# lauraset/Super-resolution-building-height-estimation

Hardware: AMD Instinct MI355X
Metric: tiles/sec (64x64x8ch->256x256 height) (higher is better)
Workload: dtype f16 operands / f32 accumulate (MFMA), f32 residual stream; 1 GPU; RRDBNet x4 (23 RRDB, 64 feat) forward_feature, batch 32 tiles/GPU, 64x64x3 -> 64x256x256 (BASELINE.json configs[1]); global_batch=32, parallelism=tile-sharded x1 (no data-path collective)

## Files before the change

super-resolution-building-height-estimation_amd/csrc/srbh_aux.hip:

```cpp
#include "srbh_internal.h"

namespace srbh {

static thread_local char g_err[512] = "";

unsigned long long g_path_counters[PATH_N] = {};
void set_error(const char* fmt, ...) {
    va_list ap;
    va_start(ap, fmt);
    vsnprintf(g_err, sizeof(g_err), fmt, ap);
    va_end(ap);
}

int hip_fail(hipError_t e, const char* what) {
    set_error("HIP error %d (%s) in %s", (int)e, hipGetErrorString(e), what);
    return (int)e;
}

__global__ void zero_words_kernel(unsigned* __restrict__ p, size_t n) {
    size_t i = (size_t)blockIdx.x * blockDim.x + threadIdx.x;
    const size_t stride = (size_t)gridDim.x * blockDim.x;
    for (; i < n; i += stride) p[i] = 0u;
}

// ... 129 lines not shown
        } else {
            const _Float16 h = (_Float16)v;
            hv[j] = __builtin_bit_cast(unsigned short, h);
        }
    }
    char* o = dst + (long)b * img_b + (long)(chunk0 + (o8 >> 2)) * plane_b + (long)(y + 1) * row_b + (x + 1) * PIX_B + (o8 & 3) * 16;
    uint4 pk = {(unsigned)hv[0] | ((unsigned)hv[1] << 16), (unsigned)hv[2] | ((unsigned)hv[3] << 16),
                (unsigned)hv[4] | ((unsigned)hv[5] << 16), (unsigned)hv[6] | ((unsigned)hv[7] << 16)};
    *(uint4*)o = pk;
}

template <int BF>
__global__ __launch_bounds__(256) void act16_channel_sum_kernel(const char* __restrict__ src, int B, int H, int W, int nchunk, int row_b,
                                                                 int plane_b, long img_b, float* __restrict__ out ) {
    __shared__ float red[32];
    if (threadIdx.x < 32) red[threadIdx.x] = 0.f;
    __syncthreads();
    const int oct = threadIdx.x & 3, pl = threadIdx.x >> 2;
    const int chunk = blockIdx.y;
    const long npix = (long)B * H * W;
    float acc[8] = {0.f, 0.f, 0.f, 0.f, 0.f, 0.f, 0.f, 0.f};
    for (long px = (long)blockIdx.x * 64 + pl; px < npix; px += (long)gridDim.x * 64) {
        const int x = (int)(px % W);
        const long r = px / W;
        const int y = (int)(r % H), b = (int)(r / H);
        const uint4 v = *(const uint4*)(src + (long)b * img_b + (long)chunk * plane_b + (long)(y + 1) * row_b + (x + 1) * PIX_B + oct * 16);
        const unsigned w4[4] = {v.x, v.y, v.z, v.w};
#pragma unroll
        for (int k = 0; k < 4; ++k) {
            if constexpr (BF) {
                acc[2 * k] += __builtin_bit_cast(float, w4[k] << 16);
                acc[2 * k + 1] += __builtin_bit_cast(float, w4[k] & 0xffff0000u);
            } else {
                acc[2 * k] += (float)__builtin_bit_cast(_Float16, (unsigned short)(w4[k] & 0xffffu));
                acc[2 * k + 1] += (float)__builtin_bit_cast(_Float16, (unsigned short)(w4[k] >> 16));
            }
        }
    }
#pragma unroll
    for (int k = 0; k < 8; ++k) {
        float a = acc[k];
#pragma unroll
        for (int m = 4; m < 64; m <<= 1) a += __shfl_xor(a, m);
        if ((threadIdx.x & 63) < 4) atomicAdd(&red[oct * 8 + k], a);
    }
    __syncthreads();
    if (threadIdx.x < 32) atomicAdd(out + chunk * 32 + threadIdx.x, red[threadIdx.x]);
}

template <int CIN, int BF16 = 0>
__global__ __launch_bounds__(256) void conv_first_kernel(const float* __restrict__ x, const float* __restrict__ w,
                                                         const float* __restrict__ bias, int B, int cin_rt, int H, int W,
                                                         float* ra, float* rb, float* rc, char* out16, int row_b,
                                                         int plane_b, long img_b) {
    extern __shared__ float s_w[];
    const int cin = CIN > 0 ? CIN : cin_rt;
    for (int u = threadIdx.x; u < cin * 9 * 64; u += 256) {
        const int oc = u & 63, k = u >> 6;
        s_w[u] = w[(long)oc * cin * 9 + k];
    }
    __syncthreads();
    const int wq = (W + 3) >> 2;
    const long idx = (long)blockIdx.x * 256 + threadIdx.x;
    const long total = (long)B * H * wq * 16;
    if (idx >= total) return;
    const int og = idx & 15;
    long r = idx >> 4;
    const int xg = r % wq; r /= wq;
    const int yy = r % H;
    const int b = r / H;
    const int x0 = xg * 4;
    float acc[4][4];
#pragma unroll
    for (int p = 0; p < 4; ++p)
#pragma unroll
        for (int q = 0; q < 4; ++q) acc[p][q] = bias ? bias[og * 4 + q] : 0.f;
    for (int ic = 0; ic < cin; ++ic) {
        const float* xp = x + ((long)b * cin + ic) * H * W;
#pragma unroll
        for (int ky = 0; ky < 3; ++ky) {
            const int sy = yy + ky - 1;
            float in[6];
#pragma unroll
            for (int j = 0; j < 6; ++j) {
                const int sx = x0 + j - 1;
                in[j] = (sy >= 0 && sy < H && sx >= 0 && sx < W) ? xp[(long)sy * W + sx] : 0.f;
            }
#pragma unroll
            for (int kx = 0; kx < 3; ++kx) {
                const float4 wv = *(const float4*)(s_w + (ic * 9 + ky * 3 + kx) * 64 + og * 4);
#pragma unroll
                for (int p = 0; p < 4; ++p) {
                    const float v = in[p + kx];
                    acc[p][0] = fmaf(v, wv.x, acc[p][0]);
                    acc[p][1] = fmaf(v, wv.y, acc[p][1]);
                    acc[p][2] = fmaf(v, wv.z, acc[p][2]);
                    acc[p][3] = fmaf(v, wv.w, acc[p][3]);
                }
            }
        }
    }
#pragma unroll
    for (int p = 0; p < 4; ++p) {
        const int xx = x0 + p;
        if (xx >= W) break;
        const long pix = ((long)b * H + yy) * W + xx;
        const float4 v4 = make_float4(acc[p][0], acc[p][1], acc[p][2], acc[p][3]);
        if (ra) *(float4*)(ra + pix * 64 + og * 4) = v4;
        if (rb) *(float4*)(rb + pix * 64 + og * 4) = v4;
// ... 201 lines not shown
            float4 row = {0.f, 0.f, 0.f, 0.f};
#pragma unroll
            for (int q = 0; q < 4; ++q) {
                const int gx = min(max(2 * ix - 1 + q, 0), 2 * W - 1);
                const float4 v = p[((long)gy * 2 * W + gx) * C4];
                row.x += wt[q] * v.x; row.y += wt[q] * v.y; row.z += wt[q] * v.z; row.w += wt[q] * v.w;
            }
            s.x += wt[a] * row.x; s.y += wt[a] * row.y; s.z += wt[a] * row.z; s.w += wt[a] * row.w;
        }
        dx[i] = s;
    }
}

extern "C" int srbh_bilinear2x_nhwc_f32(const float* x, float* out, int B, int H, int W, int C, int backward, void* stream) {
    SRBH_REQUIRE(x && out && B > 0 && H > 0 && W > 0 && C > 0 && (C & 3) == 0, "srbh_bilinear2x_nhwc_f32: bad arguments (C %% 4 == 0)");
    const long n4 = (long)B * H * W * (C / 4) * (backward ? 1 : 4);
    const int blocks = (int)((n4 + 255) / 256 < 8192 ? (n4 + 255) / 256 : 8192);
    if (backward) hipLaunchKernelGGL(bilinear2x_bwd_kernel, dim3(blocks), dim3(256), 0, (hipStream_t)stream, (const float4*)x, (float4*)out, n4, H, W, C / 4);
    else hipLaunchKernelGGL(bilinear2x_fwd_kernel, dim3(blocks), dim3(256), 0, (hipStream_t)stream, (const float4*)x, (float4*)out, n4, H, W, C / 4);
    SRBH_HIP(hipGetLastError());
    return SRBH_OK;
}

extern "C" int srbh_lrelu_bwd_f32(float* g, const float* y, float slope, long n, void* stream) {
    SRBH_REQUIRE(g && y && n > 0 && (n & 3) == 0, "srbh_lrelu_bwd_f32: bad arguments");
    const long n4 = n / 4;
    const int blocks = (int)((n4 + 255) / 256 < 4096 ? (n4 + 255) / 256 : 4096);
    hipLaunchKernelGGL(lrelu_bwd_kernel, dim3(blocks), dim3(256), 0, (hipStream_t)stream, (float4*)g, (const float4*)y, slope, n4);
    SRBH_HIP(hipGetLastError());
    return SRBH_OK;
}

extern "C" int srbh_act16_channel_sum(const void* src, int B, int H, int W, int chunks_total, int chunk0, int nchunk, int bf16, float* out,
                                      void* stream) {
    SRBH_REQUIRE(src && out && B > 0 && H > 0 && W > 0 && nchunk > 0 && chunk0 >= 0 && chunk0 + nchunk <= chunks_total, "srbh_act16_channel_sum: bad arguments");
    const Act16Geo g = act16_geo(B, chunks_total, H, W);
    if (int rc = zero_async(out, (size_t)nchunk * 32 * sizeof(float), (hipStream_t)stream)) return rc;
    const long npix = (long)B * H * W;
    const int gx = (int)((npix + 255) / 256 < 1024 ? (npix + 255) / 256 : 1024);
    const char* base = (const char*)src + (long)chunk0 * g.plane_b;
    if (bf16) hipLaunchKernelGGL(act16_channel_sum_kernel<1>, dim3(gx, nchunk), dim3(256), 0, (hipStream_t)stream, base, B, H, W, nchunk, g.row_b, g.plane_b, g.img_b, out);
    else hipLaunchKernelGGL(act16_channel_sum_kernel<0>, dim3(gx, nchunk), dim3(256), 0, (hipStream_t)stream, base, B, H, W, nchunk, g.row_b, g.plane_b, g.img_b, out);
    SRBH_HIP(hipGetLastError());
    return SRBH_OK;
}

extern "C" int srbh_conv_first_f32(const float* x, const float* w, const float* bias, int B, int cin, int H, int W,
                                   float* ra, float* rb, float* rc, void* out16, int out16_chunks_total,
                                   void* stream) {
    return srbh::conv_first_f32(x, w, bias, B, cin, H, W, ra, rb, rc, out16, out16_chunks_total, 0, stream);
}

int srbh::conv_first_f32(const float* x, const float* w, const float* bias, int B, int cin, int H, int W, float* ra, float* rb, float* rc,
                         void* out16, int out16_chunks_total, int bf16, void* stream) {
    SRBH_REQUIRE(x && w && B > 0 && cin > 0 && H > 0 && W > 0, "srbh_conv_first_f32: bad arguments");
    SRBH_REQUIRE(!out16 || out16_chunks_total >= 2, "srbh_conv_first_f32: out16 needs >= 2 chunk planes");
    Act16Geo g = act16_geo(B, out16_chunks_total > 0 ? out16_chunks_total : 2, H, W);
    SRBH_REQUIRE(cin <= 56, "srbh_conv_first_f32: at most 56 input channels (got %d)", cin);
    long total = (long)B * H * ((W + 3) / 4) * 16;
    const size_t lds = (size_t)cin * 9 * 64 * sizeof(float);
    if (cin == 3 && bf16)
        hipLaunchKernelGGL((conv_first_kernel<3, 1>), dim3((total + 255) / 256), dim3(256), lds, (hipStream_t)stream, x, w, bias,
                           B, cin, H, W, ra, rb, rc, (char*)out16, g.row_b, g.plane_b, g.img_b);
    else if (cin == 3)
        hipLaunchKernelGGL(conv_first_kernel<3>, dim3((total + 255) / 256), dim3(256), lds, (hipStream_t)stream, x, w, bias,
                           B, cin, H, W, ra, rb, rc, (char*)out16, g.row_b, g.plane_b, g.img_b);
    else if (bf16) {
        if (lds > 65536)
            SRBH_ONCE_PER_DEVICE(SRBH_HIP(hipFuncSetAttribute((const void*)conv_first_kernel<0, 1>, hipFuncAttributeMaxDynamicSharedMemorySize, 56 * 9 * 64 * 4)));
        hipLaunchKernelGGL((conv_first_kernel<0, 1>), dim3((total + 255) / 256), dim3(256), lds, (hipStream_t)stream, x, w, bias,
                           B, cin, H, W, ra, rb, rc, (char*)out16, g.row_b, g.plane_b, g.img_b);
    } else {
        if (lds > 65536)
            SRBH_ONCE_PER_DEVICE(SRBH_HIP(hipFuncSetAttribute((const void*)conv_first_kernel<0>, hipFuncAttributeMaxDynamicSharedMemorySize, 56 * 9 * 64 * 4)));
        hipLaunchKernelGGL(conv_first_kernel<0>, dim3((total + 255) / 256), dim3(256), lds, (hipStream_t)stream, x, w, bias,
                           B, cin, H, W, ra, rb, rc, (char*)out16, g.row_b, g.plane_b, g.img_b);
    }
    SRBH_HIP(hipGetLastError());
    return SRBH_OK;
}
```

super-resolution-building-height-estimation_amd/csrc/srbh_internal.h:

```cpp
#pragma once
#include <hip/hip_runtime.h>
#include <stdarg.h>
#include <stdio.h>
#include <type_traits>
#include <vector>
#include "srbh.h"

namespace srbh {

constexpr int PIX_B = 64;
constexpr int CHUNK_C = 32;
constexpr int TILE_W = 64;
constexpr int TILE_H = 8;

void set_error(const char* fmt, ...);
enum PathCounter { PATH_HCONV16 = 0, PATH_HCONV_TEMPLATE, PATH_ENTRY_FUSED, PATH_ENTRY_SPLIT, PATH_WGRAD16, PATH_WGRAD_B16_GENERIC,
                   PATH_WGRAD_F32, PATH_WGRAD_ENTRY_FUSED, PATH_WGRAD_ENTRY_SPLIT, PATH_HCONV_UP, PATH_HBWD16, PATH_HBLOCK16, PATH_N };
extern unsigned long long g_path_counters[PATH_N];
inline void count_path(int i) { ++g_path_counters[i]; }
int hconv16_wgs_cap();
int hconv_up_wgs_cap();
int hconv_entry_wgs_cap();
int hblock16_wgs_cap();
int hwgrad16_wgs_cap();
// ... 23 lines not shown
        if (!((done_ >> (dev_ & 63)) & 1ull)) {           \
            stmt;                                         \
            done_ |= 1ull << (dev_ & 63);                 \
        }                                                 \
    } while (0)

template <class P>
inline void head_set_tiles(P& p, int B, int H, int W, int th) {
    p.B = B; p.H = H; p.W = W;
    p.tiles_x = (W + TILE_W - 1) / TILE_W;
    p.tiles_per_img = p.tiles_x * ((H + th - 1) / th);
    p.ntiles = p.tiles_per_img * B;
    p.tiles_per_xcd = (p.ntiles + 7) / 8;
}
template <class P>
inline int head_walk_grid(const P& p, int cap) { return (p.tiles_per_xcd < cap / 8 ? p.tiles_per_xcd : cap / 8) * 8; }
template <int N, class F>
inline int with_const(int v, F&& f) {
    if constexpr (N == 1) return f(std::integral_constant<int, 0>{});
    else return v == N - 1 ? f(std::integral_constant<int, N - 1>{}) : with_const<N - 1>(v, f);
}
template <auto Kernel, bool RAISE_LDS = false, class P>
inline int launch(dim3 grid, int lds_bytes, hipStream_t st, const P& p) {
    if constexpr (RAISE_LDS)
        SRBH_ONCE_PER_DEVICE(SRBH_HIP(hipFuncSetAttribute((const void*)Kernel, hipFuncAttributeMaxDynamicSharedMemorySize, lds_bytes)));
    hipLaunchKernelGGL(Kernel, grid, dim3(256), lds_bytes, st, p);
    SRBH_HIP(hipGetLastError());
    return SRBH_OK;
}

struct Act16Geo {
    int row_b;
    int plane_b;
    long img_b;
    size_t total_b;
};
inline Act16Geo act16_geo(int B, int chunks, int H, int W) {
    Act16Geo g;
    g.row_b = (W + 2) * PIX_B;
    g.plane_b = (H + 2) * g.row_b;
    g.img_b = (long)chunks * g.plane_b;
    size_t slack = (size_t)(TILE_H + 4) * (size_t)((W + 2 > TILE_W + 2) ? (W + 2) : (TILE_W + 2)) * PIX_B + 8192;
    g.total_b = (size_t)B * g.img_b + slack;
    g.total_b = (g.total_b + 255) & ~(size_t)255;
    return g;
}


size_t ptrunk_aux_bytes(int B, int tiles_per_img);
size_t ptrunk_err_offset(int B, int tiles_per_img);
int ptail_run(const srbh_conv3x3_args* a, hipStream_t stream, int* used);
int ptail_wgs_cap();
int ptrunk_takes(int num_block, int H, int W, int* takes, int* ncu_out);
int ptrunk_run(const srbh_rrdbnet_desc* d, void* dense0, void* dense1, float* xr, float* xrr, int B, int H, int W,
               void* aux, hipStream_t stream, int* used, int* final_cur, long train_stride = 0, const void* mask = nullptr, long mask_stride = 0,
               bool bf16 = false);
int conv3x3_trunk_b16(const srbh_conv3x3_args* a, int out_f16, void* stream);
int conv_first_f32(const float* x, const float* w, const float* bias, int B, int cin, int H, int W, float* ra, float* rb, float* rc,
                   void* out16, int out16_chunks_total, int bf16, void* stream);


#if defined(__HIP_DEVICE_COMPILE__) || defined(__HIPCC__)
__device__ __forceinline__ void fold_stat_slots(double* stats, const int C, const int clear, double* red, double& s, double& q) {
    constexpr int NS = 64;
    const int t = threadIdx.x, V = 2 * C, G = 256 / V, v = t % V, g = t / V;
    double part = 0.0;
    if (g < G) {
        for (int k = g; k < NS; k += G) part += stats[(long)k * V + v];
        if (clear)
            for (int k = g; k < NS; k += G) stats[(long)k * V + v] = 0.0;
        red[g * V + v] = part;
    }
    __syncthreads();
    s = 0.0;
    q = 0.0;
    if (t < C)
        for (int k = 0; k < G; ++k) {
            s += red[k * V + t];
            q += red[k * V + C + t];
        }
}

__device__ __forceinline__ unsigned bf16x2_rne(float lo, float hi) {
    typedef float f2_t __attribute__((ext_vector_type(2)));
    typedef __bf16 b2_t __attribute__((ext_vector_type(2)));
    const f2_t f = {lo, hi};
    return __builtin_bit_cast(unsigned, __builtin_convertvector(f, b2_t));
}
#endif
}
```

super-resolution-building-height-estimation_amd/csrc/srbh_ptail.hip:

```cpp
#include "srbh_ptail_kernel.h"

namespace {
using namespace srbh;
using namespace srbh_k;

struct TParams {
    In16 in;
    const char* w;
    const float* bias;
    int H, W;
    int tiles_x, tiles_per_img, ntiles, tiles_per_wg;
    int lrelu;
    Out16 out16;
    float* out32;
};

constexpr int LRELU_RT = 2, OUT_16 = 1, OUT_32 = 2, OUT_RT = 3;
template <int UPS, int FULL>
constexpr int LDS_B = TAIL_LDS_B<UPS> + (FULL && UPS ? 2 * TileGeo<UPS>::UNITS * 16 : 0);

template <int UPS, int LRELU, int OUT, int FULL>
__global__ __launch_bounds__(256, 1) void ptail_kernel(const TParams p) {
    static_assert(FULL ? (LRELU != LRELU_RT && OUT != OUT_RT) : (LRELU == LRELU_RT && OUT == OUT_RT), "one general form, the rest full-tile forms");
    using G = TileGeo<UPS>;
// ... 166 lines not shown
                        for (int g = 0; g < 4; ++g) {
                            const floatx4 v = value(mb, i, g);
                            half4 h4;
#pragma unroll
                            for (int q = 0; q < 4; ++q) h4[q] = (_Float16)v[q];
                            const uint2 u = __builtin_bit_cast(uint2, h4);
                            hp[g][0] = u.x;
                            hp[g][1] = u.y;
                        }
#pragma unroll
                        for (int m = 0; m < 2; ++m) *(uintx4*)(o + (long)i * o16.row_b + (long)mb * o16.plane_b + m * 32) = pair16(hp[2 * m], hp[2 * m + 1]);
                    }
            }
            continue;
        }
        const int X = X0 + wc * 32 + l31;
#pragma unroll
        for (int i = 0; i < 4; ++i) {
            const int Y = Y0 + wr * 4 + i;
            const bool valid = (Y < p.H) && (X < p.W);
            const long pix = ((long)img * p.H + Y) * p.W + X;
#pragma unroll
            for (int mb = 0; mb < CB; ++mb) {
                unsigned hp[4][2];
#pragma unroll
                for (int g = 0; g < 4; ++g) {
                    floatx4 v;
#pragma unroll
                    for (int q = 0; q < 4; ++q) v[q] = acc[mb][i][g * 4 + q];
                    v += bias4[mb][g];
                    if (p.lrelu) {
#pragma unroll
                        for (int q = 0; q < 4; ++q) v[q] = v[q] >= 0.f ? v[q] : v[q] * 0.2f;
                    }
                    if (p.out32 && valid) *(floatx4*)(p.out32 + pix * 64 + mb * 32 + g * 8 + hi * 4) = v;
                    half4 h4;
#pragma unroll
                    for (int q = 0; q < 4; ++q) h4[q] = (_Float16)v[q];
                    const uint2 u = __builtin_bit_cast(uint2, h4);
                    hp[g][0] = u.x;
                    hp[g][1] = u.y;
                }
                if (p.out16.base) {
#pragma unroll
                    for (int m = 0; m < 2; ++m) {
                        store16_pair(p.out16, valid, img, mb, Y, X, m, hi, hp[2 * m], hp[2 * m + 1]);
                    }
                }
            }
        }
    }
}

thread_local int g_ptail_wgs_cap = 0;

thread_local int g_ptail_form_counts[SRBH_PTAIL_FORMS] = {};

template <int UPS, int LRELU, int OUT, int FULL>
int launch(const TParams& p0, hipStream_t stream) {
    static_assert(LDS_B<UPS, FULL> <= 163840, "resident weights + the input chunks must fit the 160 KiB LDS");
    constexpr auto kernel = ptail_kernel<UPS, LRELU, OUT, FULL>;
    constexpr int lds_b = LDS_B<UPS, FULL>;
    SRBH_ONCE_PER_DEVICE(SRBH_HIP(hipFuncSetAttribute((const void*)kernel, hipFuncAttributeMaxDynamicSharedMemorySize, lds_b)));
    TParams p = p0;
    int grid = 0;
    if (const int rc = tail_grid(p.ntiles, &p.tiles_per_wg, &grid)) return rc;
    hipLaunchKernelGGL(kernel, dim3(grid), dim3(256), lds_b, stream, p);
    SRBH_HIP(hipGetLastError());
    ++g_ptail_form_counts[FULL ? 1 + 4 * UPS + 2 * LRELU + (OUT == OUT_32) : 0];
    return SRBH_OK;
}

}

extern "C" int srbh_ptail_wgs_cap(int cap) {
    const int prev = g_ptail_wgs_cap;
    g_ptail_wgs_cap = cap > 0 ? cap : 0;
    return prev;
}

extern "C" int srbh_ptail_form_counts(int* counts, int n, int reset) {
    for (int i = 0; counts && i < n && i < SRBH_PTAIL_FORMS; ++i) counts[i] = g_ptail_form_counts[i];
    if (reset) for (int i = 0; i < SRBH_PTAIL_FORMS; ++i) g_ptail_form_counts[i] = 0;
    return SRBH_PTAIL_FORMS;
}

namespace srbh {

int ptail_wgs_cap() { return g_ptail_wgs_cap; }

int ptail_run(const srbh_conv3x3_args* a, hipStream_t stream, int* used) {
    *used = 0;
    const char* e = getenv("SRBH_PTAIL");
    if (e && e[0] == '0') return SRBH_OK;
    if (a->in_chunks != 2 || a->cout != 64 || a->res1 || a->res2 || a->skip) return SRBH_OK;
    if (a->out32 && a->out32_c != 64) return SRBH_OK;
    const int tiles_x = (a->W + TILE_W - 1) / TILE_W, tiles_y = (a->H + TILE_H - 1) / TILE_H;
    if (a->out16_nhwc && (!a->out16 || a->out32)) return SRBH_OK;
    if ((long)tiles_x * tiles_y * a->B < 512 && !a->out16_nhwc) return SRBH_OK;
    TParams p{};
    p.in = tail_in16(a, a->in, a->in_chunks_total, a->in_chunk0);
    p.w = (const char*)a->w;
    p.bias = a->bias;
    p.H = a->H;
    p.W = a->W;
    p.tiles_x = tiles_x;
    p.tiles_per_img = tiles_x * tiles_y;
    p.ntiles = p.tiles_per_img * a->B;
    p.lrelu = a->lrelu;
    p.out16 = tail_out16(a, a->out16, a->out16_chunks_total, a->out16_chunk0);
    p.out32 = a->out32;
    const bool full = a->H % TILE_H == 0 && a->W % TILE_W == 0 && (p.out16.base != nullptr) != (p.out32 != nullptr);
    const int rc = with_const<2>(a->upsample2x != 0, [&](auto u) {
        constexpr int UPS = decltype(u)::value;
        if (!full) return launch<UPS, LRELU_RT, OUT_RT, 0>(p, stream);
        return with_const<2>(a->lrelu != 0, [&](auto l) {
            return with_const<2>(p.out32 != nullptr, [&](auto o) { return launch<UPS, decltype(l)::value, decltype(o)::value ? OUT_32 : OUT_16, 1>(p, stream); });
        });
    });
    if (rc == SRBH_OK) *used = 1;
    return rc;
}

}
```

super-resolution-building-height-estimation_amd/csrc/srbh_ptrunk.hip:

```cpp
#include <stdlib.h>
#include <string.h>
#include <mutex>
#include "srbh_conv3x3_kernel.h"


namespace {
using namespace srbh;
using namespace srbh_k;

struct PLayer {
    const char* w;
    const float* bias;
};

struct PParams {
    char* dense[2];
    long img_b;
    int plane_b, row_b;
    float* xr;
    float* xrr;
    const PLayer* layers;
    int nlayers;
    int H, W, tiles_per_img, nblocks;
    int* prog;
    int* err;
    int* xcc;
    int force_wt;
    unsigned long long* prof;
    long dense_stride;
    int keep_all;
    int out_pixel;
    const char* mask;
    long mask_stride;
};

constexpr unsigned SPIN_LIMIT = 4u << 20;
using G = TileGeo<0>;
constexpr int IN_EX = G::UNITS * 16;
constexpr int A_STAGE_B = IN_EX + 18 * 1024, B_STAGE_B = IN_EX + 36 * 1024;
constexpr int A_BASE = IN_EX;
constexpr int A_BIAS_OFF = A_BASE + 2 * A_STAGE_B, B_BIAS_OFF = 2 * B_STAGE_B;
constexpr int P_WORD_OFF = A_BIAS_OFF + 128;
constexpr int P_LDS_B = 163840;
static_assert(P_WORD_OFF + 4 <= P_LDS_B && B_BIAS_OFF + 256 <= P_WORD_OFF, "LDS map must fit 160 KiB");
__device__ __forceinline__ int stage_off(int cb, int idx) { return cb == 1 ? A_BASE + idx * A_STAGE_B : idx * B_STAGE_B; }

#include "srbh_ptrunk3_kernel.h"

}

namespace srbh {

unsigned long long* g_ptrunk_prof = nullptr;
static int g_trunk_timing = 0;
static hipEvent_t g_trunk_ev[2];
static int g_trunk_ev_recorded = 0;
static const char* g_trunk_kernel = "none";

constexpr int MAX_BLOCKS = 64;
static size_t table_bytes() { return ((size_t)MAX_BLOCKS * 15 * sizeof(PLayer) + 255) & ~(size_t)255; }
static size_t prog_bytes(int B, int tpi) { return ((size_t)B * 2 * tpi * sizeof(int) + 255) & ~(size_t)255; }

size_t ptrunk_aux_bytes(int B, int tiles_per_img) { return table_bytes() + 2 * prog_bytes(B, tiles_per_img) + 256; }
__global__ void ptrunk_reset_kernel(int* __restrict__ prog, int* __restrict__ xcc, int* __restrict__ err, int n) {
    const int i = blockIdx.x * blockDim.x + threadIdx.x;
    if (i < n) { prog[i] = 0; xcc[i] = 0; }
    if (i == 0) *err = 0;
}

size_t ptrunk_err_offset(int B, int tiles_per_img) { return table_bytes() + prog_bytes(B, tiles_per_img); }

struct TabEntry {
    int dev;
    std::vector<char> host;
    PLayer* dptr;
};
static std::mutex g_tab_mu;
static std::vector<TabEntry> g_tabs;

static int device_table(const std::vector<PLayer>& tab, PLayer** out) {
    int dev = 0;
    SRBH_HIP(hipGetDevice(&dev));
    const size_t nb = tab.size() * sizeof(PLayer);
    std::lock_guard<std::mutex> lock(g_tab_mu);
    for (size_t i = 0; i < g_tabs.size(); ++i)
        if (g_tabs[i].dev == dev && g_tabs[i].host.size() == nb && memcmp(g_tabs[i].host.data(), tab.data(), nb) == 0) {
            *out = g_tabs[i].dptr;
            return SRBH_OK;
        }
    if (g_tabs.size() >= 16) {
        SRBH_HIP(hipFree(g_tabs.front().dptr));
        g_tabs.erase(g_tabs.begin());
    }
    TabEntry e;
    e.dev = dev;
    e.host.assign((const char*)tab.data(), (const char*)tab.data() + nb);
    SRBH_HIP(hipMalloc(&e.dptr, nb));
    SRBH_HIP(hipMemcpy(e.dptr, tab.data(), nb, hipMemcpyHostToDevice));
    *out = e.dptr;
    g_tabs.push_back(std::move(e));
    return SRBH_OK;
}

int ptrunk_takes(int num_block, int H, int W, int* takes, int* ncu_out) {
    *takes = 0;
    if (W != TILE_W || (H % TILE_H) != 0 || num_block <= 0 || num_block > MAX_BLOCKS) return SRBH_OK;
    int dev = 0;
    SRBH_HIP(hipGetDevice(&dev));
    int ncu = 0;
    SRBH_HIP(hipDeviceGetAttribute(&ncu, hipDeviceAttributeMultiprocessorCount, dev));
    if (ncu_out) *ncu_out = ncu;
    if (H / TILE_H > ncu) return SRBH_OK;
    constexpr int LDS_B = P_LDS_B;
    SRBH_ONCE_PER_DEVICE({
        SRBH_HIP(hipFuncSetAttribute((const void*)ptrunk3_kernel<0>, hipFuncAttributeMaxDynamicSharedMemorySize, LDS_B));
        SRBH_HIP(hipFuncSetAttribute((const void*)ptrunk3_kernel<1>, hipFuncAttributeMaxDynamicSharedMemorySize, LDS_B));
        SRBH_HIP(hipFuncSetAttribute((const void*)ptrunk3_kernel<0, 1>, hipFuncAttributeMaxDynamicSharedMemorySize, LDS_B));
        SRBH_HIP(hipFuncSetAttribute((const void*)ptrunk3_kernel<0, 0, 1>, hipFuncAttributeMaxDynamicSharedMemorySize, LDS_B));
    });
    int per_cu = 0;
    SRBH_HIP(hipOccupancyMaxActiveBlocksPerMultiprocessor(&per_cu, ptrunk3_kernel<0>, 256, LDS_B));
    if (per_cu < 1) return SRBH_OK;
    *takes = 1;
    return SRBH_OK;
}

int ptrunk_run(const srbh_rrdbnet_desc* d, void* dense0, void* dense1, float* xr, float* xrr, int B, int H, int W,
               void* aux, hipStream_t stream, int* used, int* final_cur, long train_stride, const void* mask, long mask_stride, bool bf16) {
    *used = 0;
    if (mask && train_stride <= 0) return SRBH_OK;
    SRBH_REQUIRE(!bf16 || (train_stride == 0 && !mask), "ptrunk_run: the bf16 form is the inference forward only");
    int ncu = 0, takes = 0;
    if (int rc = ptrunk_takes(d->num_block, H, W, &takes, &ncu)) return rc;
    if (!takes) return SRBH_OK;
    const int tpi = H / TILE_H;
    constexpr int LDS_B = P_LDS_B;
    const int nl = d->num_block * 15;
    std::vector<PLayer> tab(nl);
    int cur = 0, li = 0;
    for (int blk = 0; blk < d->num_block; ++blk)
        for (int r = 0; r < 3; ++r) {
            const srbh_conv_w* cw = d->rdb + (blk * 3 + r) * 5;
            for (int k = 0; k < 5; ++k) tab[li++] = PLayer{(const char*)cw[k].w, cw[k].bias};
            cur ^= 1;
        }
    *final_cur = cur;
    char* a = (char*)aux;
    PLayer* d_tab = nullptr;
    if (int rc = device_table(tab, &d_tab)) return rc;
    int* d_prog = (int*)(a + table_bytes());
    int* d_err = (int*)(a + ptrunk_err_offset(B, tpi));
    int* d_xcc = (int*)(a + ptrunk_err_offset(B, tpi) + 256);
    hipLaunchKernelGGL(ptrunk_reset_kernel, dim3((B * tpi + 255) / 256), dim3(256), 0, stream, d_prog, d_xcc, d_err, B * tpi);
    SRBH_HIP(hipGetLastError());
    const Act16Geo g = act16_geo(B, 6, H, W);
    int imgs_per_launch = ncu / tpi;
    if (const char* ie = getenv("SRBH_PT_IMAGES")) {
        const int cap = atoi(ie);
        if (cap > 0 && cap < imgs_per_launch) {
            const int nl_ = (B + cap - 1) / cap;
            imgs_per_launch = (B + nl_ - 1) / nl_;
        }
    }
    for (int b0 = 0; b0 < B; b0 += imgs_per_launch) {
        const int nb = (B - b0) < imgs_per_launch ? (B - b0) : imgs_per_launch;
        PParams pp;
        pp.dense_stride = train_stride;
        pp.keep_all = pp.out_pixel = train_stride > 0;
        pp.mask = mask ? (const char*)mask + (long)b0 * g.img_b : nullptr;
        pp.mask_stride = mask_stride;
        pp.dense[0] = (char*)dense0 + (long)b0 * g.img_b;
        pp.dense[1] = (train_stride > 0 ? (char*)dense0 + train_stride : (char*)dense1) + (long)b0 * g.img_b;
        pp.img_b = g.img_b;
        pp.plane_b = g.plane_b;
        pp.row_b = g.row_b;
        pp.xr = xr + (long)b0 * H * W * 64;
        pp.xrr = xrr + (long)b0 * H * W * 64;
        pp.layers = d_tab;
        pp.nlayers = nl;
        pp.H = H;
        pp.W = W;
        pp.tiles_per_img = tpi;
        pp.nblocks = nb * tpi;
        pp.prog = d_prog + b0 * tpi;
        pp.err = d_err;
        pp.xcc = d_xcc + b0 * tpi;
        {
            const char* e = getenv("SRBH_PT_WT");
            pp.force_wt = (e && atoi(e) == 1) ? 1 : 0;
        }
        if (getenv("SRBH_PT_PROF") && !bf16 && !g_ptrunk_prof)
            SRBH_HIP(hipMalloc(&g_ptrunk_prof, (size_t)ncu * MAX_BLOCKS * 15 * 6 * 8));
        pp.prof = bf16 ? nullptr : g_ptrunk_prof;
        if (g_trunk_timing && b0 == 0) SRBH_HIP(hipEventRecord(g_trunk_ev[0], stream));
        g_trunk_kernel = "ptrunk3_kernel";
        if (mask)
            hipLaunchKernelGGL((ptrunk3_kernel<0, 1>), dim3(pp.nblocks), dim3(256), LDS_B, stream, pp);
        else if (bf16)
            hipLaunchKernelGGL((ptrunk3_kernel<0, 0, 1>), dim3(pp.nblocks), dim3(256), LDS_B, stream, pp);
        else if (pp.prof)
            hipLaunchKernelGGL((ptrunk3_kernel<1>), dim3(pp.nblocks), dim3(256), LDS_B, stream, pp);
        else
            hipLaunchKernelGGL((ptrunk3_kernel<0>), dim3(pp.nblocks), dim3(256), LDS_B, stream, pp);
        SRBH_HIP(hipGetLastError());
    }
    if (g_trunk_timing) { SRBH_HIP(hipEventRecord(g_trunk_ev[1], stream)); g_trunk_ev_recorded = 1; }
    if (getenv("SRBH_PT_PROF") && g_ptrunk_prof && !bf16) {
// ... 64 lines not shown
```

super-resolution-building-height-estimation_amd/csrc/srbh_rrdbnet.hip:

```cpp
#include <stdlib.h>
#include "srbh_internal.h"

using namespace srbh;

namespace {

struct WsLayout {
    size_t d0, d1, feat, xr, xrr, u2, u3, u4, aux, total;
    size_t u2lo, u3lo;
    size_t dense_b;
};

inline size_t align256(size_t v) { return (v + 255) & ~(size_t)255; }

__global__ __launch_bounds__(256) void poison_on_error_kernel(const int* __restrict__ err, float* __restrict__ out, size_t n) {
    if (__hip_atomic_load(err, __ATOMIC_RELAXED, __HIP_MEMORY_SCOPE_AGENT) == 0) return;
    const float nan = __builtin_nanf("");
    for (size_t i = (size_t)blockIdx.x * blockDim.x + threadIdx.x; i < n; i += (size_t)gridDim.x * blockDim.x) out[i] = nan;
}

__global__ __launch_bounds__(256) void trunk_out_pixel_order_kernel(const float* __restrict__ src, float* __restrict__ dst, long nquads) {
    typedef float f4 __attribute__((ext_vector_type(4)));
    for (long i = (long)blockIdx.x * blockDim.x + threadIdx.x; i < nquads; i += (long)gridDim.x * blockDim.x) {
        const long row = i >> 10;
// ... 91 lines not shown
    L.xr = off; off = align256(off + res_b);
    L.xrr = off; off = align256(off + res_b);
    L.u2 = off; off = align256(off + act16_geo(B, 2, 2 * H, 2 * W).total_b);
    L.u3 = off; off = align256(off + act16_geo(B, 2, 4 * H, 4 * W).total_b);
    L.u4 = off;
    if (want_forward == 1) off = align256(off + act16_geo(B, 2, 4 * H, 4 * W).total_b);
    L.aux = off;
    off = align256(off + ptrunk_aux_bytes(B, tiles_per_img(H)));
    L.u2lo = L.u3lo = off;
    if (f16x2) {
        L.u2lo = off; off = align256(off + act16_geo(B, 2, 2 * H, 2 * W).total_b);
        L.u3lo = off; off = align256(off + act16_geo(B, 2, 4 * H, 4 * W).total_b);
    }
    L.total = off;
    return L;
}

}

extern "C" size_t srbh_rrdbnet_workspace_bytes(int B, int H, int W, int want_forward) {
    if (B <= 0 || H <= 0 || W <= 0) return 0;
    return ws_layout(B, H, W, want_forward).total;
}

extern "C" size_t srbh_rrdbnet_workspace_bytes_f16x2(int B, int H, int W, int want_forward) {
    if (B <= 0 || H <= 0 || W <= 0) return 0;
    return ws_layout(B, H, W, want_forward, true).total;
}

extern "C" int srbh_rrdbnet_forward(const srbh_rrdbnet_desc* d, const float* x, float* out, int B, int H, int W,
                                    int want_forward, void* ws, size_t ws_bytes, void* stream) {
    SRBH_REQUIRE(d && x && out && ws, "srbh_rrdbnet_forward: null pointer");
    SRBH_REQUIRE(B > 0 && H > 0 && W > 0, "srbh_rrdbnet_forward: bad geometry B=%d H=%d W=%d", B, H, W);
    SRBH_REQUIRE(d->num_block >= 0 && d->rdb != nullptr, "srbh_rrdbnet_forward: bad descriptor");
    const bool split = d->tail_f16x2 != 0;
    SRBH_REQUIRE(!split || (d->conv_body_lo && d->conv_up1_lo && d->conv_up2_lo && d->conv_hr_lo),
                 "srbh_rrdbnet_forward: the f16x2 mode needs the lo' packs of conv_body, conv_up1, conv_up2 and conv_hr");
    SRBH_REQUIRE(!split || want_forward != 1, "srbh_rrdbnet_forward: the f16x2 mode computes forward_feature only (want_forward 0 or 2)");
    const WsLayout L = ws_layout(B, H, W, want_forward, split);
    if (ws_bytes < L.total) {
        set_error("srbh_rrdbnet_forward: workspace %zu bytes < required %zu", ws_bytes, L.total);
        return SRBH_ERR_WORKSPACE;
    }
    char* base = (char*)ws;
    void* D[2] = {base + L.d0, base + L.d1};
    float* feat = (float*)(base + L.feat);
    float* xr = (float*)(base + L.xr);
    float* xrr = (float*)(base + L.xrr);
    void* U2 = base + L.u2;
    void* U3 = base + L.u3;
    void* U4 = base + L.u4;

    const bool bf16 = d->rdb_b16 && d->num_block > 0 && !env_off("SRBH_TRUNK_BF16");
    int rc = conv_first_f32(x, d->conv_first_w, d->conv_first_b, B, d->num_in_ch, H, W, feat, xr, xrr, D[0], 6, bf16 ? 1 : 0, stream);
    if (rc) return rc;

    int cur = 0;
    int used_persistent = 0;
    if (!env_off("SRBH_PERSISTENT")) {
        srbh_rrdbnet_desc dt = *d;
        if (bf16) dt.rdb = d->rdb_b16;
        rc = ptrunk_run(&dt, D[0], D[1], xr, xrr, B, H, W, base + L.aux, (hipStream_t)stream, &used_persistent, &cur, 0, nullptr, 0, bf16);
        if (rc) return rc;
    }
    const int n_rdb = d->num_block * 3;
    for (int i = 0; !used_persistent && i < n_rdb; ++i) {
        const srbh_conv_w* cw = (bf16 ? d->rdb_b16 : d->rdb) + i * 5;
        if ((rc = run_rdb(D[cur], D[cur ^ 1], xr, i % 3 == 2 ? xrr : nullptr, cw, B, H, W, bf16, i + 1 == n_rdb, stream))) return rc;
        cur ^= 1;
    }

    void* U2lo = base + L.u2lo;
    void* U3lo = base + L.u3lo;
    if (split && (rc = srbh_act16_split_lo(xrr, used_persistent, D[cur], 6, 0, D[cur], 6, 2, B, H, W, stream))) return rc;
    srbh_conv3x3_args a = tail_conv(D[cur], 6, d->conv_body, B, H, W, 0, 0);
    a.skip = feat;
    out_planes(a, D[cur ^ 1], 6, 0);
    if ((rc = run_tail_conv(a, split, D[cur], 6, 2, d->conv_body_lo, D[cur ^ 1], 6, 2, stream))) return rc;
    a = tail_conv(D[cur ^ 1], 6, d->conv_up1, B, 2 * H, 2 * W, 1, 1);
    out_planes(a, U2, 2, 0);
    if ((rc = run_tail_conv(a, split, D[cur ^ 1], 6, 2, d->conv_up1_lo, U2lo, 2, 0, stream))) return rc;
    a = tail_conv(U2, 2, d->conv_up2, B, 4 * H, 4 * W, 1, 1);
    out_planes(a, U3, 2, 0);
    if ((rc = run_tail_conv(a, split, U2lo, 2, 0, d->conv_up2_lo, U3lo, 2, 0, stream))) return rc;
    a = tail_conv(U3, 2, d->conv_hr, B, 4 * H, 4 * W, 0, 0);
    const bool full = want_forward && want_forward != 2 && !split;
    int out_c = 64;
    if (want_forward == 2) {
        out_planes(a, out, 2, 0);
        a.out16_nhwc = 1;
        out_c = 32;
    } else if (!full) {
        a.out32 = out; a.out32_c = 64;
    } else {
        a.lrelu = 1;
        out_planes(a, U4, 2, 0);
    }
    if ((rc = run_tail_conv(a, split, U3lo, 2, 0, d->conv_hr_lo, nullptr, 0, 0, stream))) return rc;
    if (full) {
        SRBH_REQUIRE(d->conv_last.w && d->num_out_ch >= 1 && d->num_out_ch <= 32,
                     "srbh_rrdbnet_forward: conv_last needs 1..32 output channels (got %d)", d->num_out_ch);
        a = conv_on(U4, 2, 2, d->conv_last.w, d->conv_last.bias, 32, B, 4 * H, 4 * W);
        a.out32 = out; a.out32_c = out_c = d->num_out_ch;
        if ((rc = srbh_conv3x3_f16(&a, stream))) return rc;
    }
    if (!used_persistent) return SRBH_OK;
    return poison_on_error(ptrunk_err_word(base + L.aux, B, H), out, (size_t)B * 16 * H * W * out_c, 1024, (hipStream_t)stream);
}

extern "C" int srbh_rrdbnet_trunk_out(const void* ws, size_t ws_bytes, int num_block, int B, int H, int W, int want_forward, float* out,
                                      void* stream) {
    SRBH_REQUIRE(ws && out && B > 0 && H > 0 && W > 0 && num_block >= 0, "srbh_rrdbnet_trunk_out: bad arguments");
    const WsLayout L = ws_layout(B, H, W, want_forward);
    if (ws_bytes < L.total) {
        set_error("srbh_rrdbnet_trunk_out: workspace %zu bytes < required %zu", ws_bytes, L.total);
        return SRBH_ERR_WORKSPACE;
// ... 215 lines not shown
```

Baseline: 8555 tiles/s.

## Add pipelined conv_hr fp32 tail kernel and fold trunk reset into conv_first

Adds a dedicated fp32 full-tile kernel for the final conv_hr layer. It prefetches the next tile's input chunks partway through the MFMA loop and partway through the output store loop, so staging overlaps with compute and stores. The persistent-trunk progress, xcc and error-word reset is folded into the conv_first kernel, which removes a separate launch. conv_first also skips writing xr when the persistent trunk will run. Together these cut launch overhead and stalls on the tail layer, at the cost of a larger code path and a hard requirement that the persistent trunk accept the launch.

```diff
diff --git a/super-resolution-building-height-estimation_amd/csrc/srbh_aux.hip b/super-resolution-building-height-estimation_amd/csrc/srbh_aux.hip
--- a/super-resolution-building-height-estimation_amd/csrc/srbh_aux.hip
+++ b/super-resolution-building-height-estimation_amd/csrc/srbh_aux.hip
@@ -205,9 +205,14 @@
 __global__ __launch_bounds__(256) void conv_first_kernel(const float* __restrict__ x, const float* __restrict__ w,
                                                          const float* __restrict__ bias, int B, int cin_rt, int H, int W,
                                                          float* ra, float* rb, float* rc, char* out16, int row_b,
-                                                         int plane_b, long img_b) {
+                                                         int plane_b, long img_b, const PtrunkClear clr) {
     extern __shared__ float s_w[];
     const int cin = CIN > 0 ? CIN : cin_rt;
+    if (clr.n > 0) {
+        const long i = (long)blockIdx.x * 256 + threadIdx.x;
+        if (i < clr.n) { clr.prog[i] = 0; clr.xcc[i] = 0; }
+        if (i == 0) *clr.err = 0;
+    }
     for (int u = threadIdx.x; u < cin * 9 * 64; u += 256) {
         const int oc = u & 63, k = u >> 6;
         s_w[u] = w[(long)oc * cin * 9 + k];
@@ -515,30 +520,32 @@
 }
 
 int srbh::conv_first_f32(const float* x, const float* w, const float* bias, int B, int cin, int H, int W, float* ra, float* rb, float* rc,
-                         void* out16, int out16_chunks_total, int bf16, void* stream) {
+                         void* out16, int out16_chunks_total, int bf16, void* stream, const PtrunkClear* clear) {
     SRBH_REQUIRE(x && w && B > 0 && cin > 0 && H > 0 && W > 0, "srbh_conv_first_f32: bad arguments");
     SRBH_REQUIRE(!out16 || out16_chunks_total >= 2, "srbh_conv_first_f32: out16 needs >= 2 chunk planes");
     Act16Geo g = act16_geo(B, out16_chunks_total > 0 ? out16_chunks_total : 2, H, W);
     SRBH_REQUIRE(cin <= 56, "srbh_conv_first_f32: at most 56 input channels (got %d)", cin);
     long total = (long)B * H * ((W + 3) / 4) * 16;
     const size_t lds = (size_t)cin * 9 * 64 * sizeof(float);
+    const PtrunkClear clr = clear ? *clear : PtrunkClear{};
+    SRBH_REQUIRE(clr.n == 0 || (clr.prog && clr.xcc && clr.err && clr.n <= total), "srbh_conv_first_f32: bad clear words");
     if (cin == 3 && bf16)
         hipLaunchKernelGGL((conv_first_kernel<3, 1>), dim3((total + 255) / 256), dim3(256), lds, (hipStream_t)stream, x, w, bias,
-                           B, cin, H, W, ra, rb, rc, (char*)out16, g.row_b, g.plane_b, g.img_b);
+                           B, cin, H, W, ra, rb, rc, (char*)out16, g.row_b, g.plane_b, g.img_b, clr);
     else if (cin == 3)
         hipLaunchKernelGGL(conv_first_kernel<3>, dim3((total + 255) / 256), dim3(256), lds, (hipStream_t)stream, x, w, bias,
-                           B, cin, H, W, ra, rb, rc, (char*)out16, g.row_b, g.plane_b, g.img_b);
+                           B, cin, H, W, ra, rb, rc, (char*)out16, g.row_b, g.plane_b, g.img_b, clr);
     else if (bf16) {
         if (lds > 65536)
             SRBH_ONCE_PER_DEVICE(SRBH_HIP(hipFuncSetAttribute((const void*)conv_first_kernel<0, 1>, hipFuncAttributeMaxDynamicSharedMemorySize, 56 * 9 * 64 * 4)));
         hipLaunchKernelGGL((conv_first_kernel<0, 1>), dim3((total + 255) / 256), dim3(256), lds, (hipStream_t)stream, x, w, bias,
-                           B, cin, H, W, ra, rb, rc, (char*)out16, g.row_b, g.plane_b, g.img_b);
+                           B, cin, H, W, ra, rb, rc, (char*)out16, g.row_b, g.plane_b, g.img_b, clr);
     } else {
         if (lds > 65536)
             SRBH_ONCE_PER_DEVICE(SRBH_HIP(hipFuncSetAttribute((const void*)conv_first_kernel<0>, hipFuncAttributeMaxDynamicSharedMemorySize, 56 * 9 * 64 * 4)));
         hipLaunchKernelGGL(conv_first_kernel<0>, dim3((total + 255) / 256), dim3(256), lds, (hipStream_t)stream, x, w, bias,
-                           B, cin, H, W, ra, rb, rc, (char*)out16, g.row_b, g.plane_b, g.img_b);
-    }
-    SRBH_HIP(hipGetLastError());
-    return SRBH_OK;
-}
+                           B, cin, H, W, ra, rb, rc, (char*)out16, g.row_b, g.plane_b, g.img_b, clr);
+    }
+    SRBH_HIP(hipGetLastError());
+    return SRBH_OK;
+}
diff --git a/super-resolution-building-height-estimation_amd/csrc/srbh_internal.h b/super-resolution-building-height-estimation_amd/csrc/srbh_internal.h
--- a/super-resolution-building-height-estimation_amd/csrc/srbh_internal.h
+++ b/super-resolution-building-height-estimation_amd/csrc/srbh_internal.h
@@ -99,12 +99,19 @@
 int ptail_run(const srbh_conv3x3_args* a, hipStream_t stream, int* used);
 int ptail_wgs_cap();
 int ptrunk_takes(int num_block, int H, int W, int* takes, int* ncu_out);
+struct PtrunkClear {
+    int* prog = nullptr;
+    int* xcc = nullptr;
+    int* err = nullptr;
+    int n = 0;
+};
+PtrunkClear ptrunk_clear_words(void* aux, int B, int tiles_per_img);
 int ptrunk_run(const srbh_rrdbnet_desc* d, void* dense0, void* dense1, float* xr, float* xrr, int B, int H, int W,
                void* aux, hipStream_t stream, int* used, int* final_cur, long train_stride = 0, const void* mask = nullptr, long mask_stride = 0,
-               bool bf16 = false);
+               bool bf16 = false, bool cleared = false);
 int conv3x3_trunk_b16(const srbh_conv3x3_args* a, int out_f16, void* stream);
 int conv_first_f32(const float* x, const float* w, const float* bias, int B, int cin, int H, int W, float* ra, float* rb, float* rc,
-                   void* out16, int out16_chunks_total, int bf16, void* stream);
+                   void* out16, int out16_chunks_total, int bf16, void* stream, const PtrunkClear* clear = nullptr);
 
 
 #if defined(__HIP_DEVICE_COMPILE__) || defined(__HIPCC__)
diff --git a/super-resolution-building-height-estimation_amd/csrc/srbh_ptail.hip b/super-resolution-building-height-estimation_amd/csrc/srbh_ptail.hip
--- a/super-resolution-building-height-estimation_amd/csrc/srbh_ptail.hip
+++ b/super-resolution-building-height-estimation_amd/csrc/srbh_ptail.hip
@@ -242,14 +242,145 @@
     }
 }
 
+#ifndef PTAIL_LINES_SPLIT
+#define PTAIL_LINES_SPLIT 66
+#endif
+constexpr int LINES_STORES = 128, LINES_SPLIT = PTAIL_LINES_SPLIT;
+constexpr int LINES_YOUNGER = LINES_STORES - LINES_SPLIT < 63 ? LINES_STORES - LINES_SPLIT : 63;
+static_assert(LINES_SPLIT >= 0 && LINES_SPLIT < LINES_STORES && LINES_SPLIT % 2 == 0, "the two stores of a pixel record stay together");
+
+__global__ __launch_bounds__(256, 1) void ptail_hr32_lines(const TParams p) {
+    using G = TileGeo<0>;
+    constexpr int IN_EX = G::UNITS * 16;
+    constexpr int CB = 2;
+    extern __shared__ __attribute__((aligned(16))) char smem[];
+    const int tid = threadIdx.x;
+    const int lane = tid & 63;
+    const int wave = __builtin_amdgcn_readfirstlane(tid >> 6);
+    const int l31 = lane & 31, hi = lane >> 5;
+    const int wr = wave >> 1, wc = wave & 1;
+
+    int goff[G::NJ];
+#pragma unroll
+    for (int j = 0; j < G::NJ; ++j) {
+        const int u0 = j * 256 + tid;
+        const int u = u0 < G::UNITS ? u0 : 0;
+        const int trow = u / (G::COLS * 4);
+        const int rem = u - trow * (G::COLS * 4);
+        const int pc = rem >> 2, ps = rem & 3;
+        goff[j] = trow * p.in.row_b + pc * PIX_B + ((ps ^ ((pc >> 2) & 3)) << 4);
+    }
+    const unsigned long long tail_mask = __builtin_amdgcn_ballot_w64((G::NJ - 1) * 256 + tid < G::UNITS);
+    int aoff[3][2];
+#pragma unroll
+    for (int dx = 0; dx < 3; ++dx) {
+        const int pc = wc * 32 + l31 + dx;
+#pragma unroll
+        for (int ks = 0; ks < 2; ++ks) aoff[dx][ks] = wr * 4 * G::ROW_B + pc * PIX_B + (((ks * 2 + hi) ^ ((pc >> 2) & 3)) << 4);
+    }
+
+    auto stage_chunk = [&](int t, int c) {
+        int img, Y0, X0;
+        tile_origin(t, p.tiles_per_img, p.tiles_x, img, Y0, X0);
+        const char* src0 = p.in.base + (long)img * p.in.img_b + (long)Y0 * p.in.row_b + X0 * PIX_B;
+#pragma unroll
+        for (int j = 0; j < G::NJ; ++j)
+            dma16(src0 + (long)c * p.in.plane_b + goff[j], TAIL_W_B + c * IN_EX + (j * 256 + wave * 64) * 16, j < G::NJ - 1 ? ~0ull : tail_mask);
+    };
+
+    const int t0 = blockIdx.x * p.tiles_per_wg;
+    const int t1 = (t0 + p.tiles_per_wg < p.ntiles) ? t0 + p.tiles_per_wg : p.ntiles;
+    if (t0 >= t1) return;
+#pragma unroll
+    for (int k = 0; k < 18; ++k) dma16(p.w + (wave + 4 * k) * 1024 + lane * 16, (wave + 4 * k) * 1024, ~0ull);
+    stage_chunk(t0, 0);
+    stage_chunk(t0, 1);
+    float bias1[CB];
+#pragma unroll
+    for (int mb = 0; mb < CB; ++mb) bias1[mb] = p.bias ? p.bias[mb * 32 + l31] : 0.f;
+
+    for (int t = t0; t < t1; ++t) {
+        int img, Y0, X0;
+        tile_origin(t, p.tiles_per_img, p.tiles_x, img, Y0, X0);
+        if (t == t0) asm volatile("s_waitcnt vmcnt(0)" ::: "memory");
+        else asm volatile("s_waitcnt vmcnt(%0)" ::"n"(LINES_YOUNGER) : "memory");
+        __syncthreads();
+        floatx16 acc[CB][4];
+#pragma unroll
+        for (int mb = 0; mb < CB; ++mb)
+#pragma unroll
+            for (int i = 0; i < 4; ++i)
+#pragma unroll
+                for (int r = 0; r < 16; ++r) acc[mb][i][r] = 0.f;
+        constexpr int NREAD = G::NP + 3 * CB, NMFMA = 12 * CB;
+        half8 P[2][G::NP];
+        half8 A[2][3][CB];
+        auto load_group = [&](int q, int set) {
+            const int c = q / 6, g = q - c * 6;
+            const int ks = g / 3, dx = g - ks * 3;
+            const char* sbi = smem + TAIL_W_B + c * IN_EX;
+            const char* sbw = smem + c * (36 * 1024) + lane * 16;
+#pragma unroll
+            for (int r = 0; r < G::NP; ++r) P[set][r] = *(const half8*)(sbi + aoff[dx][ks] + r * G::ROW_B);
+#pragma unroll
+            for (int dy = 0; dy < 3; ++dy)
+#pragma unroll
+                for (int mb = 0; mb < CB; ++mb)
+                    A[set][dy][mb] = *(const half8*)(sbw + ((((dy * 3 + dx) * 2 + ks) * CB + mb) << 10));
+        };
+        load_group(0, 0);
+#pragma unroll
+        for (int q = 0; q < 12; ++q) {
+            if (q + 1 < 12) load_group(q + 1, (q + 1) & 1);
+#pragma unroll
+            for (int dy = 0; dy < 3; ++dy)
+#pragma unroll
+                for (int i = 0; i < 4; ++i)
+#pragma unroll
+                    for (int mb = 0; mb < CB; ++mb)
+                        acc[mb][i] = __builtin_amdgcn_mfma_f32_32x32x16_f16(P[q & 1][i + dy], A[q & 1][dy][mb], acc[mb][i], 0, 0, 0);
+            if (q == 0) __builtin_amdgcn_sched_group_barrier(0x100, NREAD, 0);
+            if (q + 1 < 12) {
+#pragma unroll
+                for (int k = 0; k < NREAD; ++k) {
+                    __builtin_amdgcn_sched_group_barrier(0x008, 1, 0);
+                    __builtin_amdgcn_sched_group_barrier(0x100, 1, 0);
+                }
+                __builtin_amdgcn_sched_group_barrier(0x008, NMFMA - NREAD, 0);
+            } else {
+                __builtin_amdgcn_sched_group_barrier(0x008, NMFMA, 0);
+            }
+            if (q == 5) {
+                __syncthreads();
+                if (t + 1 < t1) stage_chunk(t + 1, 0);
+            }
+        }
+        __syncthreads();
+
+        const long row32 = (long)p.W * 64;
+        float* const o = p.out32 + (((long)img * p.H + Y0) * p.W + X0) * 64 + (wr * 4 * row32 + (wc * 32 + hi * 4) * 64 + l31);
+#pragma unroll
+        for (int s = 0; s < LINES_STORES; s += CB) {
+            const int i = s / 32, r = (s / 2) & 15;
+            if (s == LINES_SPLIT) {
+                if (t + 1 < t1) stage_chunk(t + 1, 1);
+            }
+#pragma unroll
+            for (int mb = 0; mb < CB; ++mb) o[i * row32 + (8 * (r >> 2) + (r & 3)) * 64 + mb * 32] = acc[mb][i][r] + bias1[mb];
+            __builtin_amdgcn_sched_barrier(0);
+        }
+    }
+}
+
 thread_local int g_ptail_wgs_cap = 0;
 
 thread_local int g_ptail_form_counts[SRBH_PTAIL_FORMS] = {};
 
-template <int UPS, int LRELU, int OUT, int FULL>
+template <int UPS, int LRELU, int OUT, int FULL, int LINES = 0>
 int launch(const TParams& p0, hipStream_t stream) {
     static_assert(LDS_B<UPS, FULL> <= 163840, "resident weights + the input chunks must fit the 160 KiB LDS");
-    constexpr auto kernel = ptail_kernel<UPS, LRELU, OUT, FULL>;
+    static_assert(!LINES || (FULL && !UPS && !LRELU && OUT == OUT_32), "ptail_hr32_lines is conv_hr's fp32 full-tile form");
+    constexpr auto kernel = LINES ? ptail_hr32_lines : ptail_kernel<UPS, LRELU, OUT, FULL>;
     constexpr int lds_b = LDS_B<UPS, FULL>;
     SRBH_ONCE_PER_DEVICE(SRBH_HIP(hipFuncSetAttribute((const void*)kernel, hipFuncAttributeMaxDynamicSharedMemorySize, lds_b)));
     TParams p = p0;
@@ -283,11 +414,15 @@
     *used = 0;
     const char* e = getenv("SRBH_PTAIL");
     if (e && e[0] == '0') return SRBH_OK;
+    const char* e32 = getenv("SRBH_PTAIL_HR32");
+    const bool hr32_lines = !(e32 && e32[0] == '0');
     if (a->in_chunks != 2 || a->cout != 64 || a->res1 || a->res2 || a->skip) return SRBH_OK;
     if (a->out32 && a->out32_c != 64) return SRBH_OK;
     const int tiles_x = (a->W + TILE_W - 1) / TILE_W, tiles_y = (a->H + TILE_H - 1) / TILE_H;
     if (a->out16_nhwc && (!a->out16 || a->out32)) return SRBH_OK;
-    if ((long)tiles_x * tiles_y * a->B < 512 && !a->out16_nhwc) return SRBH_OK;
+    long min_tiles = 512;
+    if (const char* me = getenv("SRBH_PTAIL_MIN_TILES")) min_tiles = atol(me);
+    if ((long)tiles_x * tiles_y * a->B < min_tiles && !a->out16_nhwc) return SRBH_OK;
     TParams p{};
     p.in = tail_in16(a, a->in, a->in_chunks_total, a->in_chunk0);
     p.w = (const char*)a->w;
@@ -305,7 +440,13 @@
         constexpr int UPS = decltype(u)::value;
         if (!full) return launch<UPS, LRELU_RT, OUT_RT, 0>(p, stream);
         return with_const<2>(a->lrelu != 0, [&](auto l) {
-            return with_const<2>(p.out32 != nullptr, [&](auto o) { return launch<UPS, decltype(l)::value, decltype(o)::value ? OUT_32 : OUT_16, 1>(p, stream); });
+            return with_const<2>(p.out32 != nullptr, [&](auto o) {
+                constexpr int LRELU = decltype(l)::value, OUT = decltype(o)::value ? OUT_32 : OUT_16;
+                if constexpr (!UPS && !LRELU && OUT == OUT_32) {
+                    if (hr32_lines) return launch<0, 0, OUT_32, 1, 1>(p, stream);
+                }
+                return launch<UPS, LRELU, OUT, 1>(p, stream);
+            });
         });
     });
     if (rc == SRBH_OK) *used = 1;
diff --git a/super-resolution-building-height-estimation_amd/csrc/srbh_ptrunk.hip b/super-resolution-building-height-estimation_amd/csrc/srbh_ptrunk.hip
--- a/super-resolution-building-height-estimation_amd/csrc/srbh_ptrunk.hip
+++ b/super-resolution-building-height-estimation_amd/csrc/srbh_ptrunk.hip
@@ -70,6 +70,12 @@
 
 size_t ptrunk_err_offset(int B, int tiles_per_img) { return table_bytes() + prog_bytes(B, tiles_per_img); }
 
+PtrunkClear ptrunk_clear_words(void* aux, int B, int tiles_per_img) {
+    char* a = (char*)aux;
+    return PtrunkClear{(int*)(a + table_bytes()), (int*)(a + ptrunk_err_offset(B, tiles_per_img) + 256), (int*)(a + ptrunk_err_offset(B, tiles_per_img)),
+                       B * tiles_per_img};
+}
+
 struct TabEntry {
     int dev;
     std::vector<char> host;
@@ -126,7 +132,8 @@
 }
 
 int ptrunk_run(const srbh_rrdbnet_desc* d, void* dense0, void* dense1, float* xr, float* xrr, int B, int H, int W,
-               void* aux, hipStream_t stream, int* used, int* final_cur, long train_stride, const void* mask, long mask_stride, bool bf16) {
+               void* aux, hipStream_t stream, int* used, int* final_cur, long train_stride, const void* mask, long mask_stride, bool bf16,
+               bool cleared) {
     *used = 0;
     if (mask && train_stride <= 0) return SRBH_OK;
     SRBH_REQUIRE(!bf16 || (train_stride == 0 && !mask), "ptrunk_run: the bf16 form is the inference forward only");
@@ -145,14 +152,16 @@
             cur ^= 1;
         }
     *final_cur = cur;
-    char* a = (char*)aux;
     PLayer* d_tab = nullptr;
     if (int rc = device_table(tab, &d_tab)) return rc;
-    int* d_prog = (int*)(a + table_bytes());
-    int* d_err = (int*)(a + ptrunk_err_offset(B, tpi));
-    int* d_xcc = (int*)(a + ptrunk_err_offset(B, tpi) + 256);
-    hipLaunchKernelGGL(ptrunk_reset_kernel, dim3((B * tpi + 255) / 256), dim3(256), 0, stream, d_prog, d_xcc, d_err, B * tpi);
-    SRBH_HIP(hipGetLastError());
+    const PtrunkClear clr = ptrunk_clear_words(aux, B, tpi);
+    int* const d_prog = clr.prog;
+    int* const d_err = clr.err;
+    int* const d_xcc = clr.xcc;
+    if (!cleared) {
+        hipLaunchKernelGGL(ptrunk_reset_kernel, dim3((clr.n + 255) / 256), dim3(256), 0, stream, d_prog, d_xcc, d_err, clr.n);
+        SRBH_HIP(hipGetLastError());
+    }
     const Act16Geo g = act16_geo(B, 6, H, W);
     int imgs_per_launch = ncu / tpi;
     if (const char* ie = getenv("SRBH_PT_IMAGES")) {
diff --git a/super-resolution-building-height-estimation_amd/csrc/srbh_rrdbnet.hip b/super-resolution-building-height-estimation_amd/csrc/srbh_rrdbnet.hip
--- a/super-resolution-building-height-estimation_amd/csrc/srbh_rrdbnet.hip
+++ b/super-resolution-building-height-estimation_amd/csrc/srbh_rrdbnet.hip
@@ -167,16 +167,23 @@
     void* U4 = base + L.u4;
 
     const bool bf16 = d->rdb_b16 && d->num_block > 0 && !env_off("SRBH_TRUNK_BF16");
-    int rc = conv_first_f32(x, d->conv_first_w, d->conv_first_b, B, d->num_in_ch, H, W, feat, xr, xrr, D[0], 6, bf16 ? 1 : 0, stream);
+    int persistent = 0;
+    if (!env_off("SRBH_PERSISTENT")) {
+        if (int rc0 = ptrunk_takes(d->num_block, H, W, &persistent, nullptr)) return rc0;
+    }
+    const PtrunkClear clear = persistent ? ptrunk_clear_words(base + L.aux, B, tiles_per_img(H)) : PtrunkClear{};
+    int rc = conv_first_f32(x, d->conv_first_w, d->conv_first_b, B, d->num_in_ch, H, W, feat, persistent ? nullptr : xr, xrr, D[0], 6, bf16 ? 1 : 0, stream,
+                            &clear);
     if (rc) return rc;
 
     int cur = 0;
     int used_persistent = 0;
-    if (!env_off("SRBH_PERSISTENT")) {
+    if (persistent) {
         srbh_rrdbnet_desc dt = *d;
         if (bf16) dt.rdb = d->rdb_b16;
-        rc = ptrunk_run(&dt, D[0], D[1], xr, xrr, B, H, W, base + L.aux, (hipStream_t)stream, &used_persistent, &cur, 0, nullptr, 0, bf16);
+        rc = ptrunk_run(&dt, D[0], D[1], xr, xrr, B, H, W, base + L.aux, (hipStream_t)stream, &used_persistent, &cur, 0, nullptr, 0, bf16, true);
         if (rc) return rc;
+        SRBH_REQUIRE(used_persistent, "srbh_rrdbnet_forward: the persistent trunk kernel did not take a launch that ptrunk_takes gave it");
     }
     const int n_rdb = d->num_block * 3;
     for (int i = 0; !used_persistent && i < n_rdb; ++i) {
```

Result: no change. 8585 tiles/s (median of 6 runs) (+0.4%).
